# qiaozhijian/gf-orb-slam2

Hardware: AMD Instinct MI355X
Metric: frames/sec ORB extract+match, 752x480 @2000 kp (higher is better)
Workload: dtype u8; 1 GPU; configs[2]: stereo 752x480 pair, 2000 features/image, extract L+R + stereo Hamming match; frame=one camera image (a stereo pair = 2 frames + 1 association), width=752, height=480, nfeatures=2000, levels=8, contexts_per_gpu=2, contexts_chained_after_stage=1, priming_steps=48, distinct_input_batches=4

## Files before the change

gf-orb-slam2_amd/csrc/k_blur.hip:

```cpp
#include "gfo_internal.h"
#include <stdlib.h>

#include "k_blur_dev.inc"

#ifndef GFO_BLUR_WAVES
#define GFO_BLUR_WAVES 6
#endif
__global__ __launch_bounds__(256) __attribute__((amdgpu_waves_per_eu(GFO_BLUR_WAVES, GFO_BLUR_WAVES))) void k_blur(const GfoGeom* __restrict__ gp, GfoInput in,
                                              const uint8_t* __restrict__ pyr, uint8_t* __restrict__ blur, int xcd8, int nimg)
{
    const GfoGeom& g = *gp;
    const int nb = g.blur_total_b;
    const int img = xcd8 ? (int)(blockIdx.y * 8 + (blockIdx.x & 7)) : (int)blockIdx.y;
    if (img >= nimg) return;
    const int bx = xcd8 ? (int)(blockIdx.x >> 3) : (int)blockIdx.x;
    if (bx < nb)
        blur_body<true>(g, in, pyr, blur, bx, img, threadIdx.x);
    else
        blur_body<false>(g, in, pyr, blur, bx - nb, img, threadIdx.x);
}

#ifndef BLUR_MF_TILES
#define BLUR_MF_TILES 15
#endif
typedef int gfo_v4i __attribute__((ext_vector_type(4)));

__host__ __device__ __forceinline__ int blur_mf_cols(int w) { return (w + 63) / 64; }
__host__ __device__ __forceinline__ int blur_mf_runs(int h) { return (h + 16 * BLUR_MF_TILES - 1) / (16 * BLUR_MF_TILES); }
__host__ __device__ __forceinline__ int blur_mf_blocks(int w, int h) { return (blur_mf_cols(w) * blur_mf_runs(h) + 3) / 4; }

__device__ __forceinline__ unsigned long long blur_tap_window(int o)
{
    constexpr GfoGaussTaps T = gfo_gauss_taps();
    constexpr unsigned long long TP = (unsigned long long)T.a | ((unsigned long long)T.b << 8) | ((unsigned long long)T.c << 16) | ((unsigned long long)T.d << 24) |
                                      ((unsigned long long)T.c << 32) | ((unsigned long long)T.b << 40) | ((unsigned long long)T.a << 48);
    if (o >= 8 || o <= -8) return 0ull;
    return o >= 0 ? TP >> (8 * o) : TP << (-8 * o);
}

__device__ __forceinline__ void blur_body_mfma(const GfoGeom& g, const GfoInput& in, const uint8_t* __restrict__ pyr, uint8_t* __restrict__ blur,
                                               int blk, int img, int tid)
{
    constexpr GfoGaussTaps T = gfo_gauss_taps();
    constexpr int S7 = (int)(2 * (T.a + T.b + T.c) + T.d);
    constexpr unsigned TAP7[7] = {T.a, T.b, T.c, T.d, T.c, T.b, T.a};
    static_assert(T.d <= 127 && 2 * T.c <= 127 && T.b + T.d <= 127 && 2 * T.b <= 127 && T.a + T.c <= 127, "folded taps must fit a signed byte");
    int level = 0, base = 0;
    for (;;) {
        const int nb = blur_mf_blocks(g.lv[level].w, g.lv[level].h);
        if (blk < base + nb || level + 1 >= g.nlevels) break;
        base += nb;
        level++;
    }
    const GfoLevel& L = g.lv[level];
    const int w = L.w, h = L.h;
    const int wave = __builtin_amdgcn_readfirstlane(tid >> 6), lane = tid & 63;
    const int task = (blk - base) * 4 + wave;
    const int cols = blur_mf_cols(w);
    if (task >= cols * blur_mf_runs(h)) return;
    const int run = task / cols, tc = task - run * cols;
    const int x0 = 64 * tc;
    const int r0 = run * 16 * BLUR_MF_TILES;
    const int nt = min(BLUR_MF_TILES, (h - r0 + 15) / 16);
    int pitch;
    const uint8_t* src = gfo_level_ptr(g, in, pyr, level, img, &pitch);
    uint8_t* dst = blur + (long long)img * g.blur_img_stride + L.blur_off;
    const int g4 = lane >> 4, n16 = lane & 15;
    int wp[2];
#pragma unroll
    for (int q = 0; q < 2; q++) {
        const int lo = max(0, x0 + 32 * q - 3), hi = min(w - 1, x0 + 32 * q + 34);
        const int w_min = max(0, hi - 63), w_max = max(w_min, min(lo, w - 64));
        const int a = (int)((unsigned long long)(src + w_max) & 15);
        int ws = w_max - a;
        if (ws < w_min) ws = w_max - (a & 7);
        if (ws < w_min) ws = w_max;
        wp[q] = ws;
    }
#ifdef BLUR_MF_SHARE
    const bool share = wp[1] == wp[0] + 32;
#endif
    gfo_v4i B1[4];
#pragma unroll
    for (int k = 0; k < 4; k++) {
        const int ws = wp[k >> 1];
        const int x = x0 + 16 * k + n16;
        unsigned long long blo, bhi;
        if (x >= 3 && x + 3 <= w - 1) {
            const int o = ws + 16 * g4 - (x - 3);
            blo = blur_tap_window(o); bhi = blur_tap_window(o + 8);
        } else {
            blo = 0; bhi = 0;
            if (x < w) {
#pragma unroll
                for (int d = 0; d < 7; d++) {
                    const int pos = gfo_reflect101(x + d - 3, w) - ws - 16 * g4;
                    if (pos >= 0 && pos < 8) blo += (unsigned long long)TAP7[d] << (8 * pos);
                    else if (pos >= 8 && pos < 16) bhi += (unsigned long long)TAP7[d] << (8 * (pos - 8));
                }
            }
        }
        B1[k] = gfo_v4i{(int)(unsigned)blo, (int)(unsigned)(blo >> 32), (int)(unsigned)bhi, (int)(unsigned)(bhi >> 32)};
    }
    const unsigned long long B2 = (blur_tap_window(4 * g4 - n16) & 0xFFFFFFFFull) | (blur_tap_window(4 * g4 + 16 - n16) << 32);
    const gfo_v4i C1 = {128 * S7, 128 * S7, 128 * S7, 128 * S7};
    const gfo_v4i C2lo = {128 * S7 + 32768, 128 * S7 + 32768, 128 * S7 + 32768, 128 * S7 + 32768};
    struct Raw { gfo_v4i v[2]; };
    auto load_tile = [&](int t) {
        const int y = gfo_reflect101(r0 + 16 * t - 3 + n16, h);
        const uint8_t* row = src + (long long)y * pitch + 16 * g4;
        Raw r;
#ifdef BLUR_MF_SHARE
        if (share) {
            r.v[0] = *reinterpret_cast<const gfo_v4i*>(row + wp[0]);
            r.v[1] = r.v[0];
            if (g4 >= 2) r.v[1] = *reinterpret_cast<const gfo_v4i*>(row + wp[1]);
            return r;
        }
#endif
#pragma unroll
        for (int q = 0; q < 2; q++) {
#ifdef BLUR_MF_NOLOAD
            r.v[q] = gfo_v4i{y, wp[q], y, y};
#else
            r.v[q] = *reinterpret_cast<const gfo_v4i*>(row + wp[q]);
#endif
        }
        return r;
    };
    auto pass1 = [&](const Raw& raw, unsigned* lo, unsigned* hi) {
        gfo_v4i a[2];
#pragma unroll
        for (int q = 0; q < 2; q++)
            a[q] = gfo_v4i{raw.v[q][0] ^ (int)0x80808080, raw.v[q][1] ^ (int)0x80808080, raw.v[q][2] ^ (int)0x80808080, raw.v[q][3] ^ (int)0x80808080};
#ifdef BLUR_MF_SHARE
        if (share) {
#pragma unroll
            for (int i = 0; i < 4; i++) {
#ifdef BLUR_MF_SHARE_LDS
                const int up = __builtin_amdgcn_ds_bpermute(4 * ((lane + 32) & 63), a[0][i]);
                a[1][i] = g4 < 2 ? up : a[1][i];
#else
                const auto sw = __builtin_amdgcn_permlane32_swap((unsigned)a[0][i], (unsigned)a[1][i], false, false);
                a[1][i] = (int)sw[1];
#endif
            }
        }
#endif
#pragma unroll
        for (int k = 0; k < 4; k++) {
            const gfo_v4i d = __builtin_amdgcn_mfma_i32_16x16x64_i8(a[k >> 1], B1[k], C1, 0, 0, 0);
            const unsigned x01 = __builtin_amdgcn_perm((unsigned)d[1], (unsigned)d[0], 0x05010400u);
            const unsigned x23 = __builtin_amdgcn_perm((unsigned)d[3], (unsigned)d[2], 0x05010400u);
            lo[k] = __builtin_amdgcn_perm(x23, x01, 0x05040100u) ^ 0x80808080u;
            hi[k] = __builtin_amdgcn_perm(x23, x01, 0x07060302u) ^ 0x80808080u;
        }
    };
    unsigned hlo[4], hhi[4];
    Raw raw1 = load_tile(1), raw2 = load_tile(2);
    pass1(load_tile(0), hlo, hhi);
    for (int t = 0; t < nt; t++) {
        const Raw raw = raw1;
        raw1 = raw2;
        raw2 = load_tile(t + 3);
        unsigned nlo[4], nhi[4];
        pass1(raw, nlo, nhi);
        unsigned out[4];
#pragma unroll
        for (int k = 0; k < 4; k++) {
            const gfo_v4i vlo = __builtin_amdgcn_mfma_i32_16x16x32_i8((long)((unsigned long long)hlo[k] | ((unsigned long long)nlo[k] << 32)), (long)B2, C2lo, 0, 0, 0);
            const gfo_v4i vhi = __builtin_amdgcn_mfma_i32_16x16x32_i8((long)((unsigned long long)hhi[k] | ((unsigned long long)nhi[k] << 32)), (long)B2, C1, 0, 0, 0);
            unsigned o[4];
#pragma unroll
            for (int i = 0; i < 4; i++) o[i] = min((unsigned)((vhi[i] << 8) + vlo[i]) >> 16, 255u);
            out[k] = o[0] | (o[1] << 8) | (o[2] << 16) | (o[3] << 24);
            hlo[k] = nlo[k]; hhi[k] = nhi[k];
        }
        {
            auto s0 = __builtin_amdgcn_permlane32_swap(out[0], out[2], false, false); out[0] = s0[0]; out[2] = s0[1];
            auto s1 = __builtin_amdgcn_permlane32_swap(out[1], out[3], false, false); out[1] = s1[0]; out[3] = s1[1];
            auto s2 = __builtin_amdgcn_permlane16_swap(out[0], out[1], false, false); out[0] = s2[0]; out[1] = s2[1];
            auto s3 = __builtin_amdgcn_permlane16_swap(out[2], out[3], false, false); out[2] = s3[0]; out[3] = s3[1];
        }
        const int y = r0 + 16 * t + n16;
#ifdef BLUR_MF_NOSTORE
        if (y == -12345)
#else
        if (y < h)
#endif
            *reinterpret_cast<gfo_v4i*>(dst + (long long)y * L.pitch + x0 + 16 * g4) = gfo_v4i{(int)out[0], (int)out[1], (int)out[2], (int)out[3]};
    }
}

#ifndef GFO_BLUR_MF_WAVES
#define GFO_BLUR_MF_WAVES 5
#endif
__global__ __launch_bounds__(256) __attribute__((amdgpu_waves_per_eu(GFO_BLUR_MF_WAVES, 8))) void k_blur_mfma(const GfoGeom* __restrict__ gp, GfoInput in, const uint8_t* __restrict__ pyr,
                                                                                                   uint8_t* __restrict__ blur, int xcd8, int nimg)
{
    const GfoGeom& g = *gp;
    const int img = xcd8 ? (int)(blockIdx.y * 8 + (blockIdx.x & 7)) : (int)blockIdx.y;
    if (img >= nimg) return;
    const int bx = xcd8 ? (int)(blockIdx.x >> 3) : (int)blockIdx.x;
#ifndef BLUR_MF_NOBODY
    blur_body_mfma(g, in, pyr, blur, bx, img, threadIdx.x);
#endif
}

static int blur_mfma_blocks(const gfo_ctx* c)
{
#if GFO_OCV_BLUR_ROUND == 1
    return 0;
#else
    const char* e = getenv("GFO_BLUR_MFMA");
    if (e && atoi(e) == 0) return 0;
    if (!e && c->g.lv[0].w > 896) return 0;
    int blocks = 0;
    for (int l = 0; l < c->g.nlevels; l++) {
        const int w = c->g.lv[l].w, h = c->g.lv[l].h;
        if (w < 64 || h < 1 || c->g.lv[l].pitch < 64 * blur_mf_cols(w)) return 0;
        blocks += blur_mf_blocks(w, h);
    }
    return blocks;
#endif
}

void gfo_launch_blur(gfo_ctx* c, const GfoInput& in, int nimg)
{
    gfo_prof_begin(c, ST_BLUR);
    if (c->g.total_tiles + c->g.blur_total_b > 0) {
        static const int xcd_env = getenv("GFO_BLUR_XCD") ? atoi(getenv("GFO_BLUR_XCD")) : 1;
        const int xcd8 = xcd_env && nimg >= 8 ? 1 : 0;
        const int mf = blur_mfma_blocks(c);
        const unsigned blocks = mf > 0 ? (unsigned)mf : (unsigned)(c->g.total_tiles + c->g.blur_total_b);
        const dim3 grid = xcd8 ? dim3(blocks * 8u, (unsigned)(nimg + 7) / 8u) : dim3(blocks, (unsigned)nimg);
        if (mf > 0) GFO_LAUNCH(c, k_blur_mfma, grid, dim3(256), 0, c->stream, c->d_geom, in, c->d_pyr, c->d_blur, xcd8, nimg);
        else GFO_LAUNCH(c, k_blur, grid, dim3(256), 0, c->stream, c->d_geom, in, c->d_pyr, c->d_blur, xcd8, nimg);
    }
    gfo_prof_end(c);
}

void gfo_kernels_blur(std::vector<const void*>& v) { v.push_back((const void*)k_blur); v.push_back((const void*)k_blur_mfma); }
```

gf-orb-slam2_amd/csrc/k_stereo.hip:

```cpp
#include "gfo_internal.h"
#include <stdlib.h>

#define TH_HIGH 100
#define TH_LOW 50

__device__ __forceinline__ int hamming256(const uint4 a0, const uint4 a1, const uint4 b0, const uint4 b1)
{
    return __popc(a0.x ^ b0.x) + __popc(a0.y ^ b0.y) + __popc(a0.z ^ b0.z) + __popc(a0.w ^ b0.w) +
           __popc(a1.x ^ b1.x) + __popc(a1.y ^ b1.y) + __popc(a1.z ^ b1.z) + __popc(a1.w ^ b1.w);
}

struct StereoArgs {
    const gfo_keypoint* kl;
    const uint8_t* dl;
    const gfo_keypoint* kr;
    const uint8_t* dr;
    const int* cnt_dev;
    int nl_host, nr_host;
    long long pair_stride;
    const float* scale;
    gfo_stereo_params p;
    const float* min_d;
    const float* max_d;
    long long win_stride;
    GfoStereoDev out;
    int out_stride;
    float* sx;
    unsigned* sband;
    unsigned* soi;
    uint4* sdesc;
    int* row_start;
    int* lorder;
    int* lrow_start;
    int sort_stride;
    int window;
    int nlevels;
};

#include "k_wave.inc"

__global__ __launch_bounds__(1024) void k_stereo_bucket(StereoArgs a)
{
    extern __shared__ int s_hist[];
    const int pair = blockIdx.x, tid = threadIdx.x;
    const bool left = blockIdx.y == 1;
    const int nRows = a.p.n_rows;
    int* s_part = s_hist + nRows;
    const int n = a.cnt_dev ? a.cnt_dev[2 * pair + (left ? 0 : 1)] : (left ? a.nl_host : a.nr_host);
    const gfo_keypoint* kp = (left ? a.kl : a.kr) + pair * a.pair_stride;
    const int NT = blockDim.x;
    for (int r = tid; r < nRows; r += NT) s_hist[r] = 0;
    __syncthreads();
    const long long oo = (long long)pair * a.out_stride;
    for (int i = tid; i < n; i += NT) {
        const float y = kp[i].y;
        if (!left) {
            atomicAdd(&s_hist[min(max((int)floorf(y), 0), nRows - 1)], 1);
        } else if (y < 0 || y > (float)(nRows - 1)) {
            a.out.u_right[oo + i] = -1.0f;
            a.out.depth[oo + i] = -1.0f;
            a.out.best_dist[oo + i] = -1;
            a.out.best_idx[oo + i] = -1;
            a.out.counted[oo + i] = 0;
        } else {
            atomicAdd(&s_hist[(int)y], 1);
        }
    }
    __syncthreads();
    const int chunk = (nRows + NT - 1) / NT;
    const int b0 = min(tid * chunk, nRows), e0 = min(b0 + chunk, nRows);
    int s = 0;
    for (int r = b0; r < e0; r++) s += s_hist[r];
    int total;
    int run = st_block_incl_scan(s, s_part, &total) - s;
    int* rs = (left ? a.lrow_start : a.row_start) + (long long)pair * (nRows + 1);
    for (int r = b0; r < e0; r++) {
        const int v = s_hist[r];
        rs[r] = run;
        s_hist[r] = run;
        run += v;
    }
    if (tid == 0) rs[nRows] = total;
    __syncthreads();
    const long long so = (long long)pair * a.sort_stride;
    if (left) {
        for (int i = tid; i < n; i += NT) {
            const float y = kp[i].y;
            if (!(y < 0 || y > (float)(nRows - 1))) a.lorder[so + atomicAdd(&s_hist[(int)y], 1)] = i;
        }
        return;
    }
    const uint4* dr = reinterpret_cast<const uint4*>(a.dr + pair * a.pair_stride * 32);
    for (int i = tid; i < n; i += NT) {
        const gfo_keypoint k = kp[i];
        const int b = min(max((int)floorf(k.y), 0), nRows - 1);
        const int pos = atomicAdd(&s_hist[b], 1);
        a.sx[so + pos] = k.x;
        const float rr = 2.0f * a.scale[k.octave];
        int maxr = (int)fminf((float)(nRows - 1), ceilf(k.y + rr));
        int minr = (int)fmaxf(0.0f, floorf(k.y - rr));
        if (minr > maxr) { minr = 0xFFFF; maxr = 0; }
        a.sband[so + pos] = (unsigned)minr | ((unsigned)maxr << 16);
        a.soi[so + pos] = ((unsigned)k.octave << 16) | (unsigned)i;
        a.sdesc[2 * (so + pos)] = dr[2 * i];
        a.sdesc[2 * (so + pos) + 1] = dr[2 * i + 1];
    }
}

__global__ __launch_bounds__(256) void k_stereo_match(StereoArgs a)
{
    const int wave = __builtin_amdgcn_readfirstlane(threadIdx.x >> 6), lane = threadIdx.x & 63;
    const int half = lane >> 5, hl = lane & 31;
    const int pair = blockIdx.y;
    const int nl = a.cnt_dev ? a.cnt_dev[2 * pair] : a.nl_host;
    const int iL0 = (blockIdx.x * (int)(blockDim.x >> 6) + wave) * 2;
    if (iL0 >= nl) return;
    const bool act = iL0 + half < nl;
    const int iL = min(iL0 + half, nl - 1);
    const gfo_keypoint* kl = a.kl + pair * a.pair_stride;
    const uint8_t* dl = a.dl + pair * a.pair_stride * 32;
    const long long o = (long long)pair * a.out_stride + iL;
    const long long so = (long long)pair * a.sort_stride;
    float res_u = -1.0f, res_depth = -1.0f;
    int res_dist = -1, res_idx = -1, counted = 0;

    const gfo_keypoint L = kl[iL];
    const float vL = L.y, uL = L.x;
    const int nRows = a.p.n_rows;
    const bool in_rows = !(vL < 0 || vL > (float)(nRows - 1));
    const int row = in_rows ? (int)vL : 0;
    float minD = 0.f, maxD = a.p.mbf / a.p.mb;
    if (a.min_d && a.max_d) {
        minD = a.min_d[pair * a.win_stride + iL];
        maxD = a.max_d[pair * a.win_stride + iL];
    }
    const float minU = uL - maxD, maxU = uL - minD;
    const uint4* dlp = reinterpret_cast<const uint4*>(dl + (long long)iL * 32);
    const uint4 a0 = dlp[0], a1 = dlp[1];
    const int* rs = a.row_start + (long long)pair * (nRows + 1);
    const int jb = rs[max(row - a.window, 0)], je = in_rows ? rs[min(row + a.window + 1, nRows)] : jb;
    unsigned best = ((unsigned)TH_HIGH << 16);
    bool any = false;
    for (int j = jb + hl; j < je; j += 32) {
        const unsigned band = a.sband[so + j];
        const unsigned oi = a.soi[so + j];
        const int oct = (int)(oi >> 16);
        if (row < (int)(band & 0xFFFF) || row > (int)(band >> 16)) continue;
        any = true;
        if (oct < L.octave - 1 || oct > L.octave + 1) continue;
        const float rx = a.sx[so + j];
        if (rx >= minU && rx <= maxU) {
            const unsigned dist = (unsigned)hamming256(a0, a1, a.sdesc[2 * (so + j)], a.sdesc[2 * (so + j) + 1]);
            best = min(best, (dist << 16) | (oi & 0xFFFF));
        }
    }
    const unsigned long long anym = __builtin_amdgcn_ballot_w64(any);
    const bool have_cands = ((anym >> (32 * half)) & 0xFFFFFFFFull) != 0;
    best = st_half_min(best);
    if (in_rows && have_cands && !(maxU < a.p.min_x)) {
        counted = 1;
        const int bestDist = (int)(best >> 16);
        const int bestIdxR = (int)(best & 0xFFFF);
        if (bestDist < (TH_HIGH + TH_LOW) / 2) {
            float bestuR = (a.kr + pair * a.pair_stride)[bestIdxR].x;
            float disparity = uL - bestuR;
            if (disparity >= minD && disparity < maxD) {
                if (disparity <= 0) {
                    disparity = 0.01f;
                    bestuR = (float)((double)uL - 0.01);
                }
                res_depth = a.p.mbf / disparity;
                res_u = bestuR;
                res_dist = bestDist;
                res_idx = bestIdxR;
            }
        }
    }
    if (hl == 0 && act) {
        a.out.u_right[o] = res_u;
        a.out.depth[o] = res_depth;
        a.out.best_dist[o] = res_dist;
        a.out.best_idx[o] = res_idx;
        a.out.counted[o] = (unsigned char)counted;
    }
}

#define SD_KP 1
#define SD_WAVES 8
#define SD_NT (64 * SD_WAVES)
#define SD_LIST 128
__global__ __launch_bounds__(SD_NT) void k_stereo_match_direct(StereoArgs a)
{
    extern __shared__ uint4 s_rec[];
    __shared__ float s_scale[GFO_MAX_LEVELS];
    __shared__ unsigned short s_list[SD_WAVES][SD_KP][SD_LIST];
    const int pair = blockIdx.y, tid = threadIdx.x;
    const int nl = a.cnt_dev ? a.cnt_dev[2 * pair] : a.nl_host;
    const int nr = a.cnt_dev ? a.cnt_dev[2 * pair + 1] : a.nr_host;
    if ((int)blockIdx.x * SD_WAVES * SD_KP >= nl) return;
    const int nRows = a.p.n_rows;
    const gfo_keypoint* kr = a.kr + pair * a.pair_stride;
    if (tid < GFO_MAX_LEVELS) s_scale[tid] = tid < a.nlevels ? a.scale[tid] : 0.f;
    struct LeftKp { int iL; bool valid, in_rows; float vL, uL, minD, maxD; int oct; uint4 a0, a1; } Lv[SD_KP];
    {
        const gfo_keypoint* kl = a.kl + pair * a.pair_stride;
        const uint8_t* dl = a.dl + pair * a.pair_stride * 32;
        const int w_ = __builtin_amdgcn_readfirstlane(tid >> 6);
#pragma unroll
        for (int q = 0; q < SD_KP; q++) {
            const int iL = ((int)blockIdx.x * SD_WAVES + w_) * SD_KP + q;
            Lv[q].valid = iL < nl;
            Lv[q].iL = min(iL, nl - 1);
            const gfo_keypoint L = kl[Lv[q].iL];
            Lv[q].vL = L.y; Lv[q].uL = L.x; Lv[q].oct = L.octave;
            Lv[q].in_rows = Lv[q].valid && !(L.y < 0 || L.y > (float)(nRows - 1));
            Lv[q].minD = 0.f; Lv[q].maxD = a.p.mbf / a.p.mb;
            if (a.min_d && a.max_d) {
                Lv[q].minD = a.min_d[pair * a.win_stride + Lv[q].iL];
                Lv[q].maxD = a.max_d[pair * a.win_stride + Lv[q].iL];
            }
            const uint4* dlp = reinterpret_cast<const uint4*>(dl + (long long)Lv[q].iL * 32);
            Lv[q].a0 = dlp[0]; Lv[q].a1 = dlp[1];
        }
    }
    for (int j0 = 0; j0 < nr; j0 += 4 * SD_NT) {
        float kx[4], ky[4];
        int ko[4];
#pragma unroll
        for (int u = 0; u < 4; u++) {
            const int j = min(j0 + u * SD_NT + tid, nr - 1);
            kx[u] = kr[j].x; ky[u] = kr[j].y; ko[u] = kr[j].octave;
        }
        if (j0 == 0) __syncthreads();
#pragma unroll
        for (int u = 0; u < 4; u++) {
            const int j = j0 + u * SD_NT + tid;
            if (j >= nr) continue;
            const float rr = 2.0f * s_scale[ko[u] & (GFO_MAX_LEVELS - 1)];
            int maxr = (int)fminf((float)(nRows - 1), ceilf(ky[u] + rr));
            int minr = (int)fmaxf(0.0f, floorf(ky[u] - rr));
            if (minr > maxr) { minr = 1; maxr = 0; }
            s_rec[j] = make_uint4((unsigned)minr | ((unsigned)maxr << 16), __float_as_uint(kx[u]), (unsigned)ko[u], 0u);
        }
    }
    __syncthreads();
    const int wave = __builtin_amdgcn_readfirstlane(tid >> 6), lane = tid & 63;
    const uint4* dr = reinterpret_cast<const uint4*>(a.dr + pair * a.pair_stride * 32);
    const unsigned long long lt = lane == 0 ? 0ull : (~0ull >> (64 - lane));
    unsigned row[SD_KP], nsurv[SD_KP], best[SD_KP];
    float minU[SD_KP], maxU[SD_KP];
    int octL[SD_KP];
    bool any[SD_KP], inr[SD_KP];
#pragma unroll
    for (int q = 0; q < SD_KP; q++) {
        row[q] = __builtin_amdgcn_readfirstlane(Lv[q].in_rows ? (int)Lv[q].vL : 0);
        inr[q] = Lv[q].in_rows;
        minU[q] = Lv[q].uL - Lv[q].maxD; maxU[q] = Lv[q].uL - Lv[q].minD;
        octL[q] = Lv[q].oct;
        nsurv[q] = 0; best[q] = ((unsigned)TH_HIGH << 16); any[q] = false;
    }
    auto score = [&](int q) {
        for (unsigned k = lane; k < nsurv[q]; k += 64) {
            const unsigned j = s_list[wave][q][k];
            const unsigned dist = (unsigned)hamming256(Lv[q].a0, Lv[q].a1, dr[2 * j], dr[2 * j + 1]);
            best[q] = min(best[q], (dist << 16) | j);
        }
        nsurv[q] = 0;
    };
    for (int j = lane; j - lane < nr; j += 64) {
        uint4 r = make_uint4(1u, 0u, 0u, 0u);
        if (j < nr) r = s_rec[j];
        const unsigned minr = r.x & 0xFFFFu, maxr = r.x >> 16;
        const float rx = __uint_as_float(r.y);
        const int oct = (int)r.z;
#pragma unroll
        for (int q = 0; q < SD_KP; q++) {
            const bool band = inr[q] && !(row[q] < minr || row[q] > maxr);
            any[q] = any[q] || band;
            const bool keep = band && !(oct < octL[q] - 1 || oct > octL[q] + 1) && rx >= minU[q] && rx <= maxU[q];
            const unsigned long long m = __builtin_amdgcn_ballot_w64(keep);
            if (m) {
                if (keep) s_list[wave][q][nsurv[q] + __builtin_popcountll(m & lt)] = (unsigned short)j;
                nsurv[q] += __builtin_popcountll(m);
                if (nsurv[q] > SD_LIST - 64) score(q);
            }
        }
    }
#pragma unroll
    for (int q = 0; q < SD_KP; q++) {
        if (!Lv[q].valid) continue;
        if (nsurv[q]) score(q);
        const long long o = (long long)pair * a.out_stride + Lv[q].iL;
        float res_u = -1.0f, res_depth = -1.0f;
        int res_dist = -1, res_idx = -1, counted = 0;
        const bool have_cands = __builtin_amdgcn_ballot_w64(any[q]) != 0;
        const unsigned bst = st_wave_min(best[q]);
        if (inr[q] && have_cands && !(maxU[q] < a.p.min_x)) {
            counted = 1;
            const int bestDist = (int)(bst >> 16);
            const int bestIdxR = (int)(bst & 0xFFFF);
            if (bestDist < (TH_HIGH + TH_LOW) / 2) {
                float bestuR = __uint_as_float(s_rec[bestIdxR].y);
                float disparity = Lv[q].uL - bestuR;
                if (disparity >= Lv[q].minD && disparity < Lv[q].maxD) {
                    if (disparity <= 0) {
                        disparity = 0.01f;
                        bestuR = (float)((double)Lv[q].uL - 0.01);
                    }
                    res_depth = a.p.mbf / disparity;
                    res_u = bestuR;
                    res_dist = bestDist;
                    res_idx = bestIdxR;
                }
            }
        }
        if (lane == 0) {
            a.out.u_right[o] = res_u;
            a.out.depth[o] = res_depth;
            a.out.best_dist[o] = res_dist;
            a.out.best_idx[o] = res_idx;
            a.out.counted[o] = (unsigned char)counted;
        }
    }
}

#define SR_ROWS 72
#define SR_CL 64
#ifndef SR_THREADS
#define SR_THREADS 256
#endif

__global__ __launch_bounds__(SR_THREADS) void k_stereo_match_rows(StereoArgs a, int R, int cr, int xcd8, int npairs)
{
    extern __shared__ __attribute__((aligned(16))) uint8_t sr_lds[];
    uint4* r_rec = reinterpret_cast<uint4*>(sr_lds);
    uint4* r_d0 = r_rec + cr;
    uint4* r_d1 = r_d0 + cr;
    __shared__ float l_x[SR_CL], l_minD[SR_CL], l_maxD[SR_CL];
    __shared__ int l_ro[SR_CL], l_i[SR_CL];
    __shared__ uint4 l_d0[SR_CL], l_d1[SR_CL];
    __shared__ int s_rs[SR_ROWS];
    const int tid = threadIdx.x, lane = tid & 63, half = lane >> 5, hl = lane & 31, hw = tid >> 5;
    const int pair = xcd8 ? (int)(blockIdx.y * 8 + (blockIdx.x & 7)) : (int)blockIdx.y;
    if (pair >= npairs) return;
    const int nRows = a.p.n_rows, W = a.window;
    const int r0 = (int)(xcd8 ? blockIdx.x >> 3 : blockIdx.x) * R, r1 = min(r0 + R, nRows);
    if (r0 >= nRows) return;
    const int* lrs = a.lrow_start + (long long)pair * (nRows + 1);
    const int lb = lrs[r0], le = lrs[r1];
    if (lb == le) return;
    const int* rs = a.row_start + (long long)pair * (nRows + 1);
    const int rlo = max(r0 - W, 0), rhi = min(r1 + W, nRows);
    for (int t = tid; t <= rhi - rlo; t += SR_THREADS) s_rs[t] = rs[rlo + t];
    const int jb0 = rs[rlo], nR = rs[rhi] - jb0;
    const bool staged = nR <= cr;
    const long long so = (long long)pair * a.sort_stride;
    if (staged) {
        for (int t = tid; t < nR; t += SR_THREADS) {
            const long long j = so + jb0 + t;
            const unsigned band = a.sband[j], oi = a.soi[j];
            r_rec[t] = make_uint4(band & 0xFFFFu, oi, __float_as_uint(a.sx[j]), ((band >> 16) - (band & 0xFFFFu)) | (0x10000u << (oi >> 16)));
            r_d0[t] = a.sdesc[2 * j];
            r_d1[t] = a.sdesc[2 * j + 1];
        }
    }
#if defined(SR_STOP) && SR_STOP == 1
    if (nR != 123456) return;
#endif
    const gfo_keypoint* kl = a.kl + pair * a.pair_stride;
    const uint4* dl = reinterpret_cast<const uint4*>(a.dl + pair * a.pair_stride * 32);
    const bool win = a.min_d && a.max_d;
    const float maxD0 = a.p.mbf / a.p.mb;
    for (int c0 = lb; c0 < le; c0 += SR_CL) {
        const int nc = min(SR_CL, le - c0);
        __syncthreads();
        for (int t = tid; t < nc; t += SR_THREADS) {
            const int iL = a.lorder[so + c0 + t];
            const gfo_keypoint* L = kl + iL;
            l_x[t] = L->x;
            l_ro[t] = (int)L->y | (L->octave << 16);
            l_i[t] = iL;
            l_minD[t] = win ? a.min_d[pair * a.win_stride + iL] : 0.f;
            l_maxD[t] = win ? a.max_d[pair * a.win_stride + iL] : maxD0;
            l_d0[t] = dl[2 * iL];
            l_d1[t] = dl[2 * iL + 1];
        }
        __syncthreads();
#if defined(SR_STOP) && SR_STOP == 2
        if (nR != 123456) return;
#endif
        for (int t = hw; t < nc; t += SR_THREADS / 32) {
            const int ro = l_ro[t], row = ro & 0xFFFF, octL = ro >> 16;
            const float uL = l_x[t], minD = l_minD[t], maxD = l_maxD[t];
            const float minU = uL - maxD, maxU = uL - minD;
            const uint4 a0 = l_d0[t], a1 = l_d1[t];
            const unsigned octm = ((7u << octL) >> 1) << 16;
            const int jb = s_rs[max(row - W, 0) - rlo] - jb0, je = s_rs[min(row + W + 1, nRows) - rlo] - jb0;
            unsigned best = ((unsigned)TH_HIGH << 16);
            float bx = 0.f;
            bool any = false;
            if (staged) {
                for (int j0 = jb + hl; j0 < je; j0 += 64) {
                    const int j1 = j0 + 32;
                    const bool in1 = j1 < je;
                    const uint4 rec0 = r_rec[j0], rec1 = r_rec[in1 ? j1 : j0];
                    const bool band0 = (unsigned)(row - (int)rec0.x) <= (rec0.w & 0xFFFFu);
                    const bool band1 = in1 && (unsigned)(row - (int)rec1.x) <= (rec1.w & 0xFFFFu);
                    any = any || band0 || band1;
                    const float rx0 = __uint_as_float(rec0.z), rx1 = __uint_as_float(rec1.z);
                    const bool pass0 = band0 && (rec0.w & octm) != 0 && rx0 >= minU && rx0 <= maxU;
                    const bool pass1 = band1 && (rec1.w & octm) != 0 && rx1 >= minU && rx1 <= maxU;
                    if (pass0) {
                        const unsigned key = ((unsigned)hamming256(a0, a1, r_d0[j0], r_d1[j0]) << 16) | (rec0.y & 0xFFFF);
                        if (key < best) { best = key; bx = rx0; }
                    }
                    if (pass1) {
                        const unsigned key = ((unsigned)hamming256(a0, a1, r_d0[j1], r_d1[j1]) << 16) | (rec1.y & 0xFFFF);
                        if (key < best) { best = key; bx = rx1; }
                    }
                }
            } else {
                for (int j = jb + hl; j < je; j += 32) {
                    const long long g = so + jb0 + j;
                    const unsigned band = a.sband[g], oi = a.soi[g];
                    if (row < (int)(band & 0xFFFF) || row > (int)(band >> 16)) continue;
                    any = true;
                    const int oct = (int)(oi >> 16);
                    if (oct < octL - 1 || oct > octL + 1) continue;
                    const float rx = a.sx[g];
                    if (rx >= minU && rx <= maxU) {
                        const unsigned key = ((unsigned)hamming256(a0, a1, a.sdesc[2 * g], a.sdesc[2 * g + 1]) << 16) | (oi & 0xFFFF);
                        if (key < best) { best = key; bx = rx; }
                    }
                }
            }
            const unsigned long long anym = __builtin_amdgcn_ballot_w64(any);
            const bool have_cands = ((anym >> (32 * half)) & 0xFFFFFFFFull) != 0;
            unsigned red = best;
            red = st_half_min(red);
            const unsigned long long own = __builtin_amdgcn_ballot_w64(best == red && red < ((unsigned)TH_HIGH << 16));
            const unsigned ownh = (unsigned)(own >> (32 * half));
            float bestuR = __shfl(bx, 32 * half + (ownh ? __ffs((int)ownh) - 1 : 0));
            float res_u = -1.0f, res_depth = -1.0f;
            int res_dist = -1, res_idx = -1, counted = 0;
            if (have_cands && !(maxU < a.p.min_x)) {
                counted = 1;
                const int bestDist = (int)(red >> 16);
                if (bestDist < (TH_HIGH + TH_LOW) / 2) {
                    float disparity = uL - bestuR;
                    if (disparity >= minD && disparity < maxD) {
                        if (disparity <= 0) {
                            disparity = 0.01f;
                            bestuR = (float)((double)uL - 0.01);
                        }
                        res_depth = a.p.mbf / disparity;
                        res_u = bestuR;
                        res_dist = bestDist;
                        res_idx = (int)(red & 0xFFFF);
                    }
                }
            }
#if defined(SR_STOP) && SR_STOP == 3
            if (res_dist != 123456) continue;
#endif
            if (hl == 0) {
                const long long o = (long long)pair * a.out_stride + l_i[t];
                a.out.u_right[o] = res_u;
                a.out.depth[o] = res_depth;
                a.out.best_dist[o] = res_dist;
                a.out.best_idx[o] = res_idx;
                a.out.counted[o] = (unsigned char)counted;
            }
        }
    }
}

__device__ __forceinline__ void stereo_cut_pair(const int* __restrict__ cnt_dev, int nl_host, const GfoStereoDev& out, int out_stride, int pair,
                                                int* hist, int* s_part, int* s_med, int* s_drop, int* s_cnt,
                                                float* __restrict__ h_u, float* __restrict__ h_d, int* __restrict__ h_nm)
{
    const int tid = threadIdx.x, NT = blockDim.x;
    const int nl = cnt_dev ? cnt_dev[2 * pair] : nl_host;
    const long long o = (long long)pair * out_stride;
    if (tid < 128) hist[tid] = 0;
    if (tid == 0) *s_drop = 0, *s_cnt = 0, *s_med = 1 << 30;
    __syncthreads();
    int mine = 0;
    for (int i = tid; i < nl; i += NT) {
        const int d = out.best_dist[o + i];
        if (d >= 0) atomicAdd(&hist[d], 1);
        mine += out.counted[o + i];
    }
    if (mine) atomicAdd(s_cnt, mine);
    __syncthreads();
    int ndi;
    int h = 0;
    h = tid < 128 ? hist[tid] : 0;
    const int incl = st_block_incl_scan(h, s_part, &ndi);
    if (tid < 128 && ndi > 0 && incl > ndi / 2) atomicMin(s_med, tid);
    __syncthreads();
    if (ndi == 0) {
        if (h_u)
            for (int i = tid; i < nl; i += NT) { h_u[o + i] = out.u_right[o + i]; h_d[o + i] = out.depth[o + i]; }
        if (tid == 0) {
            out.nmatched[pair] = *s_cnt;
            if (h_nm) h_nm[pair] = *s_cnt;
        }
        return;
    }
    const float thDist = 1.5f * 1.4f * (float)*s_med;
    int drop = 0;
    for (int i = tid; i < nl; i += NT) {
        const int d = out.best_dist[o + i];
        const bool cut = d >= 0 && !((float)d < thDist);
        if (cut) {
            out.u_right[o + i] = -1.0f;
            out.depth[o + i] = -1.0f;
            drop++;
        }
        if (h_u) {
            h_u[o + i] = cut ? -1.0f : out.u_right[o + i];
            h_d[o + i] = cut ? -1.0f : out.depth[o + i];
        }
    }
    if (drop) atomicAdd(s_drop, drop);
    __syncthreads();
    if (tid == 0) {
        out.nmatched[pair] = *s_cnt - *s_drop;
        if (h_nm) h_nm[pair] = *s_cnt - *s_drop;
    }
}

__global__ __launch_bounds__(1024) void k_stereo_cut(const int* __restrict__ cnt_dev, int nl_host, GfoStereoDev out,
                                                     int out_stride)
{
    __shared__ int hist[128];
    __shared__ int s_part[16];
    __shared__ int s_med, s_drop, s_cnt;
    stereo_cut_pair(cnt_dev, nl_host, out, out_stride, blockIdx.x, hist, s_part, &s_med, &s_drop, &s_cnt, nullptr, nullptr, nullptr);
}

__global__ __launch_bounds__(1024) void k_pack_results_cut(GfoPack p)
{
    if ((int)blockIdx.x < p.cut_pairs) {
        __shared__ int hist[128];
        __shared__ int s_part[16];
        __shared__ int s_med, s_drop, s_cnt;
        stereo_cut_pair(p.cut_cnt_dev, p.cut_nl_host, p.cut_out, p.cut_out_stride, blockIdx.x, hist, s_part, &s_med, &s_drop, &s_cnt,
                        p.h_u_right, p.h_depth, p.h_nmatched);
        return;
    }
    const int t = ((int)blockIdx.x - p.cut_pairs) * 1024 + threadIdx.x, stride = ((int)gridDim.x - p.cut_pairs) * 1024;
    for (int s = 0; s < p.nseg; s++)
        for (int i = t; i < p.n16[s]; i += stride) p.dst[s][i] = p.src[s][i];
}

void gfo_launch_pack_cut(gfo_ctx* c, const GfoPack& p, hipStream_t st)
{
    int total = 0;
    for (int s_ = 0; s_ < p.nseg; s_++) total += p.n16[s_];
    const int copy_blocks = (total + 4095) / 4096 > 0 ? (total + 4095) / 4096 : 1;
    GFO_LAUNCH(c, k_pack_results_cut, dim3(p.cut_pairs + copy_blocks), dim3(1024), 0, st, p);
}

struct SadArgs {
    StereoArgs s;
    const GfoGeom* g;
    GfoInput in;
    const uint8_t* pyr;
    const float* inv_scale;
};

__global__ __launch_bounds__(256) void k_stereo_match_sad(SadArgs A)
{
    const StereoArgs& a = A.s;
    const GfoGeom& g = *A.g;
    const int wave = __builtin_amdgcn_readfirstlane(threadIdx.x >> 6), lane = threadIdx.x & 63;
    const int pair = blockIdx.y;
    const int iL = blockIdx.x * 4 + wave;
    const int nl = a.cnt_dev[2 * pair];
    if (iL >= nl) return;
    const gfo_keypoint* kl = a.kl + pair * a.pair_stride;
    const gfo_keypoint* kr = a.kr + pair * a.pair_stride;
    const uint8_t* dl = a.dl + pair * a.pair_stride * 32;
    const long long o = (long long)pair * a.out_stride + iL;
    const long long so = (long long)pair * a.sort_stride;
    float res_u = -1.0f, res_depth = -1.0f;
    int res_dist = -1, res_idx = -1;
    const gfo_keypoint L = kl[iL];
    const float vL = L.y, uL = L.x;
    const int nRows = a.p.n_rows;
    const int row = (int)vL;
    const float minD = 0.f, maxD = a.p.mbf / a.p.mb;
    const float minU = uL - maxD, maxU = uL - minD;
    if (row >= 0 && row <= nRows - 1 && !(maxU < 0)) {
        const uint4* dlp = reinterpret_cast<const uint4*>(dl + (long long)iL * 32);
        const uint4 a0 = dlp[0], a1 = dlp[1];
        const int* rs = a.row_start + (long long)pair * (nRows + 1);
        const int jb = rs[max(row - a.window, 0)], je = rs[min(row + a.window + 1, nRows)];
        unsigned best = ((unsigned)TH_HIGH << 16);
        for (int j = jb + lane; j < je; j += 64) {
            const unsigned band = a.sband[so + j];
            const unsigned oi = a.soi[so + j];
            const int oct = (int)(oi >> 16);
            if (row < (int)(band & 0xFFFF) || row > (int)(band >> 16)) continue;
            if (oct < L.octave - 1 || oct > L.octave + 1) continue;
            const float rx = a.sx[so + j];
            if (rx >= minU && rx <= maxU) {
                const unsigned dist = (unsigned)hamming256(a0, a1, a.sdesc[2 * (so + j)], a.sdesc[2 * (so + j) + 1]);
                best = min(best, (dist << 16) | (oi & 0xFFFF));
            }
        }
        best = st_wave_min(best);
        const int bestDist = (int)(best >> 16), bestIdxR = (int)(best & 0xFFFF);
        if (bestDist < (TH_HIGH + TH_LOW) / 2) {
            const int lvl = L.octave;
            const float uR0 = kr[bestIdxR].x;
            const float sfac = A.inv_scale[lvl];
            const float scaleduL = roundf(uL * sfac), scaledvL = roundf(vL * sfac), scaleduR0 = roundf(uR0 * sfac);
            const int w = 5, LL = 5;
            int pl, prr;
            const uint8_t* IL = gfo_level_ptr(g, A.in, A.pyr, lvl, 2 * pair, &pl);
            const uint8_t* IR = gfo_level_ptr(g, A.in, A.pyr, lvl, 2 * pair + 1, &prr);
            const int cu = (int)scaleduL, cv = (int)scaledvL, cr = (int)scaleduR0;
            const float iniu = scaleduR0 + LL - w, endu = scaleduR0 + LL + w + 1;
            if (!(iniu < 0 || endu >= (float)g.lv[lvl].w)) {
                const int ilc = IL[(long long)cv * pl + cu];
                int acc[11];
#pragma unroll
                for (int k = 0; k < 11; k++) acc[k] = 0;
                for (int p0 = 0; p0 < 121; p0 += 64) {
                    const int p = p0 + lane;
                    if (p < 121) {
                        const int dy = p / 11 - w, dx = p - (p / 11) * 11 - w;
                        const int il = (int)IL[(long long)(cv + dy) * pl + cu + dx] - ilc;
                        const uint8_t* rrow = IR + (long long)(cv + dy) * prr + cr + dx;
                        const uint8_t* rcen = IR + (long long)cv * prr + cr;
#pragma unroll
                        for (int k = 0; k < 11; k++) {
                            const int ir = (int)rrow[k - LL] - (int)rcen[k - LL];
                            acc[k] += abs(il - ir);
                        }
                    }
                }
#pragma unroll
                for (int k = 0; k < 11; k++) acc[k] = st_wave_sum(acc[k]);
                int sadBest = 2147483647, bestinc = 0;
#pragma unroll
                for (int k = 0; k < 11; k++)
                    if ((float)acc[k] < (float)sadBest) { sadBest = acc[k]; bestinc = k - LL; }
                if (!(bestinc == -LL || bestinc == LL)) {
                    float d1 = 0.f, d2 = 0.f, d3 = 0.f;
#pragma unroll
                    for (int k = 1; k < 10; k++)
                        if (k - LL == bestinc) { d1 = (float)acc[k - 1]; d2 = (float)acc[k]; d3 = (float)acc[k + 1]; }
                    const float deltaR = (d1 - d3) / (2.0f * (d1 + d3 - 2.0f * d2));
                    if (!(deltaR < -1 || deltaR > 1)) {
                        float bestuR = g.lv[lvl].scale * ((float)scaleduR0 + (float)bestinc + deltaR);
                        float disparity = uL - bestuR;
                        if (disparity >= minD && disparity < maxD) {
                            if (disparity <= 0) { disparity = 0.01f; bestuR = (float)((double)uL - 0.01); }
                            res_depth = a.p.mbf / disparity;
                            res_u = bestuR;
                            res_dist = sadBest;
                            res_idx = bestIdxR;
                        }
                    }
                }
            }
        }
    }
    if (lane == 0) {
        a.out.u_right[o] = res_u;
        a.out.depth[o] = res_depth;
        a.out.best_dist[o] = res_dist;
        a.out.best_idx[o] = res_idx;
        a.out.counted[o] = res_dist >= 0 ? 1 : 0;
    }
}

__global__ __launch_bounds__(256) void k_stereo_cut_sad(const int* __restrict__ cnt_dev, GfoStereoDev out, int out_stride)
{
    __shared__ int hist[256];
    __shared__ int s_hi, s_rank, s_med, s_drop, s_n;
    const int pair = blockIdx.x, tid = threadIdx.x;
    const int nl = cnt_dev[2 * pair];
    const long long o = (long long)pair * out_stride;
    hist[tid] = 0;
    if (tid == 0) s_drop = 0, s_n = 0;
    __syncthreads();
    int mine = 0;
    for (int i = tid; i < nl; i += 256) {
        const int d = out.best_dist[o + i];
        if (d >= 0) { atomicAdd(&hist[min(d >> 8, 255)], 1); mine++; }
    }
    if (mine) atomicAdd(&s_n, mine);
    __syncthreads();
    const int ndi = s_n;
    if (ndi == 0) { if (tid == 0) out.nmatched[pair] = 0; return; }
    if (tid == 0) {
        int acc = 0, b = 0;
        for (; b < 256; b++) { if (acc + hist[b] > ndi / 2) break; acc += hist[b]; }
        s_hi = b;
        s_rank = ndi / 2 - acc;
    }
    __syncthreads();
    const int hi = s_hi;
    __syncthreads();
    hist[tid] = 0;
    __syncthreads();
    for (int i = tid; i < nl; i += 256) {
        const int d = out.best_dist[o + i];
        if (d >= 0 && min(d >> 8, 255) == hi) atomicAdd(&hist[d & 255], 1);
    }
    __syncthreads();
    if (tid == 0) {
        int acc = 0, b = 0;
        for (; b < 256; b++) { acc += hist[b]; if (acc > s_rank) break; }
        s_med = (hi << 8) | b;
    }
    __syncthreads();
    const float thDist = 1.5f * 1.4f * (float)s_med;
    int drop = 0;
    for (int i = tid; i < nl; i += 256) {
        const int d = out.best_dist[o + i];
        if (d >= 0 && !((float)d < thDist)) {
            out.u_right[o + i] = -1.0f;
            out.depth[o + i] = -1.0f;
            drop++;
        }
    }
    if (drop) atomicAdd(&s_drop, drop);
    __syncthreads();
    if (tid == 0) out.nmatched[pair] = ndi - s_drop;
}

void gfo_launch_stereo_sad(gfo_ctx* c, const GfoStereoLaunch& s, const GfoInput& in, const float* d_inv_scale)
{
    SadArgs A{};
    StereoArgs& a = A.s;
    a.kl = s.kl; a.dl = s.dl; a.kr = s.kr; a.dr = s.dr;
    a.cnt_dev = s.cnt_dev; a.nl_host = 0; a.nr_host = 0;
    a.pair_stride = s.pair_stride_kp;
    a.scale = s.d_scale;
    a.p = s.p;
    a.min_d = nullptr; a.max_d = nullptr; a.win_stride = 0;
    a.out = s.out; a.out_stride = s.out_stride;
    a.sx = s.sort.sx; a.sband = reinterpret_cast<unsigned*>(s.sort.sy); a.soi = s.sort.soi; a.sdesc = reinterpret_cast<uint4*>(s.sort.sdesc);
    a.row_start = s.sort.row_start;
    a.lorder = nullptr; a.lrow_start = nullptr;
    a.sort_stride = s.sort_stride;
    a.window = s.window;
    A.g = c->d_geom;
    A.in = in;
    A.pyr = c->d_pyr;
    A.inv_scale = d_inv_scale;
    gfo_prof_begin(c, ST_STEREO_BUCKET);
    GFO_LAUNCH(c, k_stereo_bucket, dim3(s.npairs), dim3(1024), (size_t)(s.p.n_rows + 256) * sizeof(int), c->stream, a);
    gfo_prof_end(c);
    gfo_prof_begin(c, ST_STEREO);
    GFO_LAUNCH(c, k_stereo_match_sad, dim3((s.out_stride + 3) / 4, s.npairs), dim3(256), 0, c->stream, A);
    gfo_prof_end(c);
    gfo_prof_begin(c, ST_STEREO_CUT);
    GFO_LAUNCH(c, k_stereo_cut_sad, dim3(s.npairs), dim3(256), 0, c->stream, s.cnt_dev, s.out, s.out_stride);
    gfo_prof_end(c);
}

int gfo_stereo_window(const float* scale, int nlevels)
{
    float mx = 0.f;
    for (int l = 0; l < nlevels; l++) mx = scale[l] > mx ? scale[l] : mx;
    return (int)ceilf(2.0f * mx) + 1;
}

void gfo_launch_stereo(gfo_ctx* c, const GfoStereoLaunch& s)
{
    StereoArgs a{};
    a.kl = s.kl; a.dl = s.dl; a.kr = s.kr; a.dr = s.dr;
    a.cnt_dev = s.cnt_dev; a.nl_host = s.nl_host; a.nr_host = s.nr_host;
    a.pair_stride = s.pair_stride_kp;
    a.scale = s.d_scale;
    a.p = s.p;
    a.min_d = s.min_d; a.max_d = s.max_d; a.win_stride = s.win_stride;
    a.out = s.out; a.out_stride = s.out_stride;
    a.sx = s.sort.sx; a.sband = reinterpret_cast<unsigned*>(s.sort.sy); a.soi = s.sort.soi; a.sdesc = reinterpret_cast<uint4*>(s.sort.sdesc);
    a.row_start = s.sort.row_start;
    a.sort_stride = s.sort_stride;
    a.window = s.window;
    a.nlevels = s.nlevels;
    const int max_nl = s.cnt_dev ? s.out_stride : s.nl_host;
    if (max_nl <= 0) {
        (void)hipMemsetAsync(s.out.nmatched, 0, sizeof(int) * s.npairs, c->stream);
        return;
    }
    const int rows_env = getenv("GFO_STEREO_ROWS") ? atoi(getenv("GFO_STEREO_ROWS")) : -1;
    int R = rows_env > 0 ? rows_env : 8;
    if (R > 32) R = 32;
    const bool rows_form = rows_env != 0 && (s.npairs >= 4 || rows_env > 0) && s.sort.lorder && s.p.n_rows <= 65535 && R + 2 * s.window + 2 <= SR_ROWS;
    const char* direct_env = getenv("GFO_STEREO_DIRECT");
    const int max_nr = s.cnt_dev ? s.out_stride : s.nr_host;
    const bool direct = !rows_form && rows_env < 0 && !(direct_env && direct_env[0] == '0') && s.npairs <= 3 && max_nr > 0 && max_nr <= 3584 && s.nlevels > 0 &&
                        s.p.n_rows <= 65535;
    if (direct) {
        gfo_prof_begin(c, ST_STEREO);
        GFO_LAUNCH(c, k_stereo_match_direct, dim3((max_nl + SD_WAVES * SD_KP - 1) / (SD_WAVES * SD_KP), s.npairs), dim3(SD_NT), (size_t)max_nr * sizeof(uint4), c->stream, a);
        gfo_prof_end(c);
        if (!s.cut_in_pack) {
            gfo_prof_begin(c, ST_STEREO_CUT);
            GFO_LAUNCH(c, k_stereo_cut, dim3(s.npairs), dim3(1024), 0, c->stream, s.cnt_dev, s.nl_host, s.out, s.out_stride);
            gfo_prof_end(c);
        }
        return;
    }
    a.lorder = rows_form ? s.sort.lorder : nullptr;
    a.lrow_start = rows_form ? s.sort.lrow_start : nullptr;
    gfo_prof_begin(c, ST_STEREO_BUCKET);
    static const int bt_env = getenv("GFO_STEREO_BUCKET_THREADS") ? atoi(getenv("GFO_STEREO_BUCKET_THREADS")) : 0;
    static const int ct_env = getenv("GFO_STEREO_CUT_THREADS") ? atoi(getenv("GFO_STEREO_CUT_THREADS")) : 0;
    const int bucket_threads = bt_env == 256 || bt_env == 512 || bt_env == 1024 ? bt_env : (s.npairs >= 32 ? 512 : 1024);
    const int cut_threads = ct_env == 256 || ct_env == 512 || ct_env == 1024 ? ct_env : (s.npairs >= 32 ? 256 : 1024);
    GFO_LAUNCH(c, k_stereo_bucket, dim3(s.npairs, rows_form ? 2 : 1), dim3(bucket_threads), (size_t)(s.p.n_rows + 256) * sizeof(int), c->stream, a);
    gfo_prof_end(c);
    gfo_prof_begin(c, ST_STEREO);
    if (rows_form) {
        static const int cr_env = getenv("GFO_STEREO_CR") ? atoi(getenv("GFO_STEREO_CR")) : 0;
        const int per_row8 = (8 * max_nl + s.p.n_rows - 1) / s.p.n_rows;
        int cr = cr_env > 0 ? cr_env : ((2 * per_row8 * (R + 2 * s.window) / 8 + 63) & ~63);
        cr = cr < 64 ? 64 : (cr > 1024 ? 1024 : cr);
        static const int xcd_env = getenv("GFO_STEREO_XCD") ? atoi(getenv("GFO_STEREO_XCD")) : 1;
        const int xcd8 = xcd_env && s.npairs >= 8 ? 1 : 0;
        const unsigned bands = (unsigned)((s.p.n_rows + R - 1) / R);
        const dim3 grid = xcd8 ? dim3(bands * 8u, (unsigned)(s.npairs + 7) / 8u) : dim3(bands, (unsigned)s.npairs);
        GFO_LAUNCH(c, k_stereo_match_rows, grid, dim3(SR_THREADS), (size_t)cr * 48, c->stream, a, R, cr, xcd8, s.npairs);
    } else {
        static const int snw_env = getenv("GFO_STEREO_WAVES") ? atoi(getenv("GFO_STEREO_WAVES")) : 4;
        const int snw = snw_env < 1 ? 1 : (snw_env > 4 ? 4 : snw_env);
        dim3 grid((max_nl + 2 * snw - 1) / (2 * snw), s.npairs);
        GFO_LAUNCH(c, k_stereo_match, grid, dim3(64 * snw), 0, c->stream, a);
    }
    gfo_prof_end(c);
    if (s.cut_in_pack) return;
    gfo_prof_begin(c, ST_STEREO_CUT);
    GFO_LAUNCH(c, k_stereo_cut, dim3(s.npairs), dim3(cut_threads), 0, c->stream, s.cnt_dev, s.nl_host, s.out, s.out_stride);
    gfo_prof_end(c);
}

void gfo_kernels_stereo(std::vector<const void*>& v)
{
    v.push_back((const void*)k_stereo_bucket); v.push_back((const void*)k_stereo_match); v.push_back((const void*)k_stereo_match_rows);
    v.push_back((const void*)k_stereo_cut); v.push_back((const void*)k_stereo_match_sad); v.push_back((const void*)k_stereo_cut_sad);
    v.push_back((const void*)k_stereo_match_direct); v.push_back((const void*)k_pack_results_cut);
}
```

gf-orb-slam2_amd/csrc/k_wave.inc:

```
__device__ __forceinline__ unsigned st_row_min(unsigned v)
{
    v = min(v, (unsigned)__builtin_amdgcn_update_dpp(0, (int)v, 0xB1, 0xF, 0xF, true));
    v = min(v, (unsigned)__builtin_amdgcn_update_dpp(0, (int)v, 0x4E, 0xF, 0xF, true));
    v = min(v, (unsigned)__builtin_amdgcn_update_dpp(0, (int)v, 0x141, 0xF, 0xF, true));
    v = min(v, (unsigned)__builtin_amdgcn_update_dpp(0, (int)v, 0x140, 0xF, 0xF, true));
    return v;
}
__device__ __forceinline__ unsigned st_half_min(unsigned v)
{
    v = st_row_min(v);
    return min(v, (unsigned)__builtin_amdgcn_ds_swizzle((int)v, 0x401F));
}
__device__ __forceinline__ unsigned st_wave_min(unsigned v)
{
    v = st_half_min(v);
    return min((unsigned)__builtin_amdgcn_readlane((int)v, 0), (unsigned)__builtin_amdgcn_readlane((int)v, 32));
}
__device__ __forceinline__ int st_wave_sum(int v)
{
    v += __builtin_amdgcn_update_dpp(0, v, 0xB1, 0xF, 0xF, true);
    v += __builtin_amdgcn_update_dpp(0, v, 0x4E, 0xF, 0xF, true);
    v += __builtin_amdgcn_update_dpp(0, v, 0x141, 0xF, 0xF, true);
    v += __builtin_amdgcn_update_dpp(0, v, 0x140, 0xF, 0xF, true);
    v += __builtin_amdgcn_ds_swizzle(v, 0x401F);
    return __builtin_amdgcn_readlane(v, 0) + __builtin_amdgcn_readlane(v, 32);
}

__device__ __forceinline__ int st_wave_incl_scan(int v)
{
    v += __builtin_amdgcn_update_dpp(0, v, 0x111, 0xF, 0xF, false);
    v += __builtin_amdgcn_update_dpp(0, v, 0x112, 0xF, 0xF, false);
    v += __builtin_amdgcn_update_dpp(0, v, 0x114, 0xF, 0xF, false);
    v += __builtin_amdgcn_update_dpp(0, v, 0x118, 0xF, 0xF, false);
    v += __builtin_amdgcn_update_dpp(0, v, 0x142, 0xA, 0xF, false);
    v += __builtin_amdgcn_update_dpp(0, v, 0x143, 0xC, 0xF, false);
    return v;
}

__device__ __forceinline__ int st_block_incl_scan(int v, int* s_part, int* total)
{
    const int lane = threadIdx.x & 63, wave = threadIdx.x >> 6, nw = blockDim.x >> 6;
    const int incl = st_wave_incl_scan(v);
    if (lane == 63) s_part[wave] = incl;
    __syncthreads();
    int base = 0, tot = 0;
    for (int w = 0; w < nw; w++) {
        const int t = s_part[w];
        if (w < wave) base += t;
        tot += t;
    }
    __syncthreads();
    *total = tot;
    return base + incl;
}
```

Before: 295,100 frames/s.

## Use 16-lane groups in stereo row matching and cheaper MFMA blur packing

The stereo row-matching kernel now handles each left keypoint with a 16-lane group instead of a 32-lane half wave, doubling keypoints in flight per wave. The per-group reduction becomes a DPP row-min plus row-or, replacing the ds_swizzle, ballot and shuffle sequence. The MFMA blur kernel packs its outputs with byte permutes and saturating 16-bit adds, and stops loading tiles past the end of a run. A static cached env read becomes a per-call getenv, which adds host overhead; the narrower groups also give each keypoint less parallelism over candidates.

```diff
diff --git a/gf-orb-slam2_amd/csrc/k_blur.hip b/gf-orb-slam2_amd/csrc/k_blur.hip
--- a/gf-orb-slam2_amd/csrc/k_blur.hip
+++ b/gf-orb-slam2_amd/csrc/k_blur.hip
@@ -24,6 +24,11 @@
 #define BLUR_MF_TILES 15
 #endif
 typedef int gfo_v4i __attribute__((ext_vector_type(4)));
+typedef unsigned short gfo_v2u16 __attribute__((ext_vector_type(2)));
+#ifdef BLUR_MF_V1
+#define BLUR_MF_V1_LOADS
+#define BLUR_MF_V1_PACK
+#endif
 
 __host__ __device__ __forceinline__ int blur_mf_cols(int w) { return (w + 63) / 64; }
 __host__ __device__ __forceinline__ int blur_mf_runs(int h) { return (h + 16 * BLUR_MF_TILES - 1) / (16 * BLUR_MF_TILES); }
@@ -157,12 +162,22 @@
         }
     };
     unsigned hlo[4], hhi[4];
+#ifdef BLUR_MF_V1_LOADS
     Raw raw1 = load_tile(1), raw2 = load_tile(2);
     pass1(load_tile(0), hlo, hhi);
     for (int t = 0; t < nt; t++) {
         const Raw raw = raw1;
         raw1 = raw2;
         raw2 = load_tile(t + 3);
+#else
+    Raw raw1 = load_tile(1), raw2 = raw1;
+    if (nt >= 2) raw2 = load_tile(2);
+    pass1(load_tile(0), hlo, hhi);
+    for (int t = 0; t < nt; t++) {
+        const Raw raw = raw1;
+        raw1 = raw2;
+        if (t + 3 <= nt) raw2 = load_tile(t + 3);
+#endif
         unsigned nlo[4], nhi[4];
         pass1(raw, nlo, nhi);
         unsigned out[4];
@@ -170,10 +185,20 @@
         for (int k = 0; k < 4; k++) {
             const gfo_v4i vlo = __builtin_amdgcn_mfma_i32_16x16x32_i8((long)((unsigned long long)hlo[k] | ((unsigned long long)nlo[k] << 32)), (long)B2, C2lo, 0, 0, 0);
             const gfo_v4i vhi = __builtin_amdgcn_mfma_i32_16x16x32_i8((long)((unsigned long long)hhi[k] | ((unsigned long long)nhi[k] << 32)), (long)B2, C1, 0, 0, 0);
+#ifdef BLUR_MF_V1_PACK
             unsigned o[4];
 #pragma unroll
             for (int i = 0; i < 4; i++) o[i] = min((unsigned)((vhi[i] << 8) + vlo[i]) >> 16, 255u);
             out[k] = o[0] | (o[1] << 8) | (o[2] << 16) | (o[3] << 24);
+#else
+            const gfo_v2u16 h01 = __builtin_bit_cast(gfo_v2u16, __builtin_amdgcn_perm((unsigned)vhi[1], (unsigned)vhi[0], 0x05040100u));
+            const gfo_v2u16 h23 = __builtin_bit_cast(gfo_v2u16, __builtin_amdgcn_perm((unsigned)vhi[3], (unsigned)vhi[2], 0x05040100u));
+            const gfo_v2u16 l01 = __builtin_bit_cast(gfo_v2u16, __builtin_amdgcn_perm((unsigned)vlo[1], (unsigned)vlo[0], 0x06050201u));
+            const gfo_v2u16 l23 = __builtin_bit_cast(gfo_v2u16, __builtin_amdgcn_perm((unsigned)vlo[3], (unsigned)vlo[2], 0x06050201u));
+            const unsigned u01 = __builtin_bit_cast(unsigned, __builtin_elementwise_add_sat(h01, l01));
+            const unsigned u23 = __builtin_bit_cast(unsigned, __builtin_elementwise_add_sat(h23, l23));
+            out[k] = __builtin_amdgcn_perm(u23, u01, 0x07050301u);
+#endif
             hlo[k] = nlo[k]; hhi[k] = nhi[k];
         }
         {
diff --git a/gf-orb-slam2_amd/csrc/k_stereo.hip b/gf-orb-slam2_amd/csrc/k_stereo.hip
--- a/gf-orb-slam2_amd/csrc/k_stereo.hip
+++ b/gf-orb-slam2_amd/csrc/k_stereo.hip
@@ -329,6 +329,12 @@
 #ifndef SR_THREADS
 #define SR_THREADS 256
 #endif
+#ifndef SR_GROUP
+#define SR_GROUP 16
+#endif
+#if SR_GROUP != 16 && SR_GROUP != 32
+#error "SR_GROUP is 16 or 32"
+#endif
 
 __global__ __launch_bounds__(SR_THREADS) void k_stereo_match_rows(StereoArgs a, int R, int cr, int xcd8, int npairs)
 {
@@ -340,7 +346,8 @@
     __shared__ int l_ro[SR_CL], l_i[SR_CL];
     __shared__ uint4 l_d0[SR_CL], l_d1[SR_CL];
     __shared__ int s_rs[SR_ROWS];
-    const int tid = threadIdx.x, lane = tid & 63, half = lane >> 5, hl = lane & 31, hw = tid >> 5;
+    const int tid = threadIdx.x, lane = tid & 63;
+    const int gl = lane & (SR_GROUP - 1), gsh = lane & (64 - SR_GROUP), gw = tid / SR_GROUP;
     const int pair = xcd8 ? (int)(blockIdx.y * 8 + (blockIdx.x & 7)) : (int)blockIdx.y;
     if (pair >= npairs) return;
     const int nRows = a.p.n_rows, W = a.window;
@@ -389,7 +396,7 @@
 #if defined(SR_STOP) && SR_STOP == 2
         if (nR != 123456) return;
 #endif
-        for (int t = hw; t < nc; t += SR_THREADS / 32) {
+        for (int t = gw; t < nc; t += SR_THREADS / SR_GROUP) {
             const int ro = l_ro[t], row = ro & 0xFFFF, octL = ro >> 16;
             const float uL = l_x[t], minD = l_minD[t], maxD = l_maxD[t];
             const float minU = uL - maxD, maxU = uL - minD;
@@ -400,8 +407,8 @@
             float bx = 0.f;
             bool any = false;
             if (staged) {
-                for (int j0 = jb + hl; j0 < je; j0 += 64) {
-                    const int j1 = j0 + 32;
+                for (int j0 = jb + gl; j0 < je; j0 += 2 * SR_GROUP) {
+                    const int j1 = j0 + SR_GROUP;
                     const bool in1 = j1 < je;
                     const uint4 rec0 = r_rec[j0], rec1 = r_rec[in1 ? j1 : j0];
                     const bool band0 = (unsigned)(row - (int)rec0.x) <= (rec0.w & 0xFFFFu);
@@ -420,7 +427,7 @@
                     }
                 }
             } else {
-                for (int j = jb + hl; j < je; j += 32) {
+                for (int j = jb + gl; j < je; j += SR_GROUP) {
                     const long long g = so + jb0 + j;
                     const unsigned band = a.sband[g], oi = a.soi[g];
                     if (row < (int)(band & 0xFFFF) || row > (int)(band >> 16)) continue;
@@ -435,12 +442,18 @@
                 }
             }
             const unsigned long long anym = __builtin_amdgcn_ballot_w64(any);
-            const bool have_cands = ((anym >> (32 * half)) & 0xFFFFFFFFull) != 0;
+#if SR_GROUP == 32
+            const bool have_cands = ((anym >> gsh) & 0xFFFFFFFFull) != 0;
             unsigned red = best;
             red = st_half_min(red);
             const unsigned long long own = __builtin_amdgcn_ballot_w64(best == red && red < ((unsigned)TH_HIGH << 16));
-            const unsigned ownh = (unsigned)(own >> (32 * half));
-            float bestuR = __shfl(bx, 32 * half + (ownh ? __ffs((int)ownh) - 1 : 0));
+            const unsigned ownh = (unsigned)(own >> gsh);
+            float bestuR = __shfl(bx, gsh + (ownh ? __ffs((int)ownh) - 1 : 0));
+#else
+            const bool have_cands = ((unsigned)(anym >> gsh) & 0xFFFFu) != 0;
+            const unsigned red = st_row_min(best);
+            float bestuR = __uint_as_float(st_row_or(best == red ? __float_as_uint(bx) : 0u));
+#endif
             float res_u = -1.0f, res_depth = -1.0f;
             int res_dist = -1, res_idx = -1, counted = 0;
             if (have_cands && !(maxU < a.p.min_x)) {
@@ -463,7 +476,7 @@
 #if defined(SR_STOP) && SR_STOP == 3
             if (res_dist != 123456) continue;
 #endif
-            if (hl == 0) {
+            if (gl == 0) {
                 const long long o = (long long)pair * a.out_stride + l_i[t];
                 a.out.u_right[o] = res_u;
                 a.out.depth[o] = res_depth;
@@ -823,7 +836,7 @@
     gfo_prof_end(c);
     gfo_prof_begin(c, ST_STEREO);
     if (rows_form) {
-        static const int cr_env = getenv("GFO_STEREO_CR") ? atoi(getenv("GFO_STEREO_CR")) : 0;
+        const int cr_env = getenv("GFO_STEREO_CR") ? atoi(getenv("GFO_STEREO_CR")) : 0;
         const int per_row8 = (8 * max_nl + s.p.n_rows - 1) / s.p.n_rows;
         int cr = cr_env > 0 ? cr_env : ((2 * per_row8 * (R + 2 * s.window) / 8 + 63) & ~63);
         cr = cr < 64 ? 64 : (cr > 1024 ? 1024 : cr);
diff --git a/gf-orb-slam2_amd/csrc/k_wave.inc b/gf-orb-slam2_amd/csrc/k_wave.inc
--- a/gf-orb-slam2_amd/csrc/k_wave.inc
+++ b/gf-orb-slam2_amd/csrc/k_wave.inc
@@ -4,6 +4,14 @@
     v = min(v, (unsigned)__builtin_amdgcn_update_dpp(0, (int)v, 0x4E, 0xF, 0xF, true));
     v = min(v, (unsigned)__builtin_amdgcn_update_dpp(0, (int)v, 0x141, 0xF, 0xF, true));
     v = min(v, (unsigned)__builtin_amdgcn_update_dpp(0, (int)v, 0x140, 0xF, 0xF, true));
+    return v;
+}
+__device__ __forceinline__ unsigned st_row_or(unsigned v)
+{
+    v |= (unsigned)__builtin_amdgcn_update_dpp(0, (int)v, 0xB1, 0xF, 0xF, true);
+    v |= (unsigned)__builtin_amdgcn_update_dpp(0, (int)v, 0x4E, 0xF, 0xF, true);
+    v |= (unsigned)__builtin_amdgcn_update_dpp(0, (int)v, 0x141, 0xF, 0xF, true);
+    v |= (unsigned)__builtin_amdgcn_update_dpp(0, (int)v, 0x140, 0xF, 0xF, true);
     return v;
 }
 __device__ __forceinline__ unsigned st_half_min(unsigned v)
```

After: 298,600 frames/s (median of 3 runs). About the same (+1.2%).
